# argumentcomputer/lurk-beta

Hardware: NVIDIA H100
Metric: Lurk iterations proved/sec (fib rc=100, Nova IVC) (higher is better)
Workload: dtype u32x8 (254-bit Montgomery integers)

## Files before the change

include/lurk_b200.h:

```cpp
#ifndef LURK_B200_H
#define LURK_B200_H

#include <stddef.h>
#include <stdint.h>

#ifdef __cplusplus
extern "C" {
#endif

#define LURK_FIELD_BN254_FR 0
#define LURK_FIELD_BN254_FQ 1
#define LURK_FIELD_PALLAS_FQ 2
#define LURK_FIELD_PALLAS_FP 3

#define LURK_CURVE_BN254_G1 0
#define LURK_CURVE_GRUMPKIN 1
#define LURK_CURVE_PALLAS 2
#define LURK_CURVE_VESTA 3

#define LURK_FMT_CANONICAL 0
#define LURK_FMT_MONTGOMERY 1

#define LURK_OK 0
#define LURK_ERR_ARG (-1)
// ... 29 lines not shown
int lurk_bitdecomp_witness_batch_dev(int field_id, const void *d_values, size_t n, void *d_blocks, int fmt,
                                     void *stream);

#define LURK_DAG_TUPLE2 2
#define LURK_DAG_TUPLE3 3
#define LURK_DAG_TUPLE4 4
#define LURK_DAG_COMPACT 5
#define LURK_DAG_COMMITMENT 6
typedef struct lurk_dag_node {
    uint8_t kind;
    uint8_t reserved;
    uint16_t tag[4];
    uint32_t child[4];
} lurk_dag_node;
int lurk_dag_hash(int field_id, const lurk_dag_node *nodes, size_t n, const uint8_t *atom_digests,
                  size_t n_atoms, uint8_t *out_digests);
typedef struct lurk_dag_plan {
    uint64_t nodes, levels, max_width;
    uint64_t est_gpu_us;
    uint64_t est_cpu_core_us;
    int use_gpu;
} lurk_dag_plan;
int lurk_dag_hash_plan(const lurk_dag_node *nodes, size_t n, size_t n_atoms, lurk_dag_plan *plan);

typedef struct lurk_msm_ctx lurk_msm_ctx;
int lurk_msm_ctx_create(int curve_id, const uint8_t *bases_affine, size_t n, int fmt, lurk_msm_ctx **out);
int lurk_msm_ctx_create_dev(int curve_id, const void *d_bases_mont, size_t n, lurk_msm_ctx **out);
void lurk_msm_ctx_destroy(lurk_msm_ctx *ctx);
int lurk_msm_ctx_info(lurk_msm_ctx *ctx, int *curve_id, size_t *n);
int lurk_msm_ctx_run(lurk_msm_ctx *ctx, const uint8_t *scalars, size_t n, int fmt, uint8_t out_xyz[96]);
int lurk_msm_ctx_run_dev(lurk_msm_ctx *ctx, const void *d_scalars, size_t n, int fmt, uint8_t out_xyz[96],
                         void *stream);
int lurk_msm_ctx_precompute(lurk_msm_ctx *ctx);
int lurk_msm_ctx_launch_dev(lurk_msm_ctx *ctx, const void *d_scalars, size_t n, int fmt, void *stream);
int lurk_msm_ctx_finish(lurk_msm_ctx *ctx, uint8_t out_xyz[96]);
int lurk_msm_ctx_clone(lurk_msm_ctx *ctx, lurk_msm_ctx **out);
int lurk_msm_ctx_set_profiling(lurk_msm_ctx *ctx, int enable);
int lurk_msm_ctx_last_profile(lurk_msm_ctx *ctx, float *accumulate_ms, unsigned *kernel_launches);
int lurk_msm(int curve_id, const uint8_t *bases_affine, const uint8_t *scalars, size_t n, int fmt,
             uint8_t out_xyz[96]);
int lurk_synthetic_bases(int curve_id, uint64_t start, size_t n, int fmt, uint8_t *bases_out);
int lurk_point_sum(int curve_id, const uint8_t *points_xyz, size_t count, int fmt, uint8_t out_xyz[96]);

size_t lurk_ck_size(size_t num_cons, size_t num_vars, size_t ck_floor);
int lurk_ck_generate(int curve_id, const uint8_t *label, size_t label_len, size_t n, int fmt, uint8_t *bases_out);
int lurk_ck_generate_dev(int curve_id, const uint8_t *label, size_t label_len, size_t n, void *d_bases_mont, void *stream);
int lurk_ck_generate_range_dev(int curve_id, const uint8_t *label, size_t label_len, size_t first, size_t n, void *d_bases_mont,
                               void *stream);
int lurk_hash_to_curve_batch(int curve_id, const char *domain_prefix, const uint8_t *messages, size_t msg_len, size_t n, int fmt,
                             uint8_t *points_out);
int lurk_hash_to_curve_batch_dev(int curve_id, const char *domain_prefix, const void *d_messages, size_t msg_len, size_t n,
                                 void *d_points, int fmt, void *stream);
int lurk_ck_powers_dev(int curve_id, const uint8_t g[64], const uint8_t beta[32], size_t n, void *d_bases_mont, int fmt, void *stream);
int lurk_shake256(const uint8_t *in, size_t in_len, uint8_t *out, size_t out_len);

typedef int (*lurk_challenge_fn)(void *user, int round, const uint8_t *message, size_t message_len, uint8_t challenge_out[32]);
#define LURK_SUMCHECK_QUAD 0
#define LURK_SUMCHECK_CUBIC 1
int lurk_sumcheck_prove_dev(int field_id, int kind, void *const *d_polys, int num_rounds, const uint8_t claim[32],
                            lurk_challenge_fn challenge, void *user, uint8_t *round_evals, uint8_t *challenges, uint8_t *final_evals,
                            int fmt, void *stream);
int lurk_sumcheck_prove_batch_dev(int field_id, int kind, int n_instances, void *const *d_polys, const int *num_rounds,
                                  const uint8_t *claims, const uint8_t *coeffs, lurk_challenge_fn challenge, void *user,
                                  uint8_t *round_evals, uint8_t *challenges, uint8_t *final_evals, int fmt, void *stream);
int lurk_eq_evals_dev(int field_id, const uint8_t *tau, int num_vars, void *d_out, int fmt, void *stream);
int lurk_inner_product_dev(int field_id, const void *d_a, const void *d_b, size_t n, uint8_t out[32], int fmt, void *stream);
int lurk_ipa_fold_scalars_dev(int field_id, void *d_a, size_t n, const uint8_t x[32], const uint8_t y[32], int fmt, void *stream);
int lurk_ipa_fold_bases_dev(int curve_id, void *d_bases_mont, size_t n, const uint8_t x[32], const uint8_t y[32], int fmt, void *stream);
int lurk_ipa_prove_dev(int curve_id, lurk_msm_ctx *ck, const uint8_t ck_c[64], void *d_a, void *d_b, int log_n,
                       lurk_challenge_fn challenge, void *user, uint8_t *L_out, uint8_t *R_out, uint8_t a_final[32], uint8_t b_final[32],
                       int fmt, void *stream);
// ... 199 lines not shown
```

lurk-beta_b200/_capi.py:

```python
import ctypes as C
import os

_HERE = os.path.dirname(os.path.abspath(__file__))
LIB_PATH = os.path.join(_HERE, "liblurk_b200.so")

FIELD_BN254_FR, FIELD_BN254_FQ, FIELD_PALLAS_FQ, FIELD_PALLAS_FP = 0, 1, 2, 3
CURVE_BN254_G1, CURVE_GRUMPKIN, CURVE_PALLAS, CURVE_VESTA = 0, 1, 2, 3
FMT_CANONICAL, FMT_MONTGOMERY = 0, 1
OK, ERR_ARG, ERR_CUDA, ERR_OOM, ERR_RANGE, ERR_NOGPU, ERR_ORDER = 0, -1, -2, -3, -4, -5, -6


class LurkError(RuntimeError):
    def __init__(self, code, msg):
        super().__init__(f"liblurk_b200 error {code}: {msg}")
        self.code = code


class DagNode(C.Structure):
    _fields_ = [("kind", C.c_uint8), ("reserved", C.c_uint8), ("tag", C.c_uint16 * 4), ("child", C.c_uint32 * 4)]


class DagPlan(C.Structure):
    _fields_ = [("nodes", C.c_uint64), ("levels", C.c_uint64), ("max_width", C.c_uint64), ("est_gpu_us", C.c_uint64),
                ("est_cpu_core_us", C.c_uint64), ("use_gpu", C.c_int)]
# ... 67 lines not shown
class RecursiveVerdict(C.Structure):
    _fields_ = [("bad_rows", C.c_uint64), ("first_bad_row", C.c_uint64), ("u_ok", C.c_int), ("comm_W_ok", C.c_int), ("comm_E_ok", C.c_int)]


PROTOTYPES = {
    "lurk_last_error": (C.c_char_p, []),
    "lurk_version": (_i, []),
    "lurk_device_count": (_i, []),
    "lurk_field_modulus": (_i, [_i, _vp]),
    "lurk_poseidon_hash_batch": (_i, [_i, _i, _vp, _sz, _vp]),
    "lurk_poseidon_hash_batch_mont": (_i, [_i, _i, _vp, _sz, _vp]),
    "lurk_poseidon_hash_batch_dev": (_i, [_i, _i, _vp, _sz, _vp, _i, _vp]),
    "lurk_poseidon_constants": (_i, [_i, _i, C.POINTER(_i), C.POINTER(_i), _vp, _vp]),
    "lurk_poseidon_witness_block": (_sz, [_i, _i]),
    "lurk_poseidon_witness_batch": (_i, [_i, _i, _vp, _sz, _vp, _i]),
    "lurk_poseidon_witness_batch_dev": (_i, [_i, _i, _vp, _sz, _vp, _i, _vp]),
    "lurk_poseidon_witness_scatter_dev": (_i, [_i, _i, _vp, _sz, _vp, _vp, _i, _vp]),
    "lurk_bitdecomp_witness_scatter_dev": (_i, [_i, _vp, _sz, _vp, _vp, _i, _vp]),
    "lurk_bitdecomp_witness_block": (_sz, [_i]),
    "lurk_bitdecomp_witness_batch": (_i, [_i, _vp, _sz, _vp, _i]),
    "lurk_bitdecomp_witness_batch_dev": (_i, [_i, _vp, _sz, _vp, _i, _vp]),
    "lurk_dag_hash": (_i, [_i, _vp, _sz, _vp, _sz, _vp]),
    "lurk_dag_hash_plan": (_i, [_vp, _sz, _sz, C.POINTER(DagPlan)]),
    "lurk_msm_ctx_create": (_i, [_i, _vp, _sz, _i, C.POINTER(_vp)]),
    "lurk_msm_ctx_create_dev": (_i, [_i, _vp, _sz, C.POINTER(_vp)]),
    "lurk_msm_ctx_destroy": (None, [_vp]),
    "lurk_msm_ctx_run": (_i, [_vp, _vp, _sz, _i, _vp]),
    "lurk_msm_ctx_run_dev": (_i, [_vp, _vp, _sz, _i, _vp, _vp]),
    "lurk_msm": (_i, [_i, _vp, _vp, _sz, _i, _vp]),
    "lurk_msm_ctx_launch_dev": (_i, [_vp, _vp, _sz, _i, _vp]),
    "lurk_msm_ctx_finish": (_i, [_vp, _vp]),
    "lurk_msm_ctx_clone": (_i, [_vp, C.POINTER(_vp)]),
    "lurk_msm_ctx_precompute": (_i, [_vp]),
    "lurk_msm_ctx_set_profiling": (_i, [_vp, _i]),
    "lurk_msm_ctx_last_profile": (_i, [_vp, C.POINTER(C.c_float), C.POINTER(C.c_uint)]),
    "lurk_point_sum": (_i, [_i, _vp, _sz, _i, _vp]),
    "lurk_synthetic_bases": (_i, [_i, C.c_uint64, _sz, _i, _vp]),
    "lurk_ck_size": (_sz, [_sz, _sz, _sz]),
    "lurk_ck_generate": (_i, [_i, _vp, _sz, _sz, _i, _vp]),
    "lurk_ck_generate_dev": (_i, [_i, _vp, _sz, _sz, _vp, _vp]),
    "lurk_ck_generate_range_dev": (_i, [_i, _vp, _sz, _sz, _sz, _vp, _vp]),
    "lurk_hash_to_curve_batch": (_i, [_i, C.c_char_p, _vp, _sz, _sz, _i, _vp]),
    "lurk_hash_to_curve_batch_dev": (_i, [_i, C.c_char_p, _vp, _sz, _sz, _vp, _i, _vp]),
    "lurk_shake256": (_i, [_vp, _sz, _vp, _sz]),
    "lurk_sumcheck_prove_dev": (_i, [_i, _i, C.POINTER(_vp), _i, _vp, CHALLENGE_FN, _vp, _vp, _vp, _vp, _i, _vp]),
    "lurk_sumcheck_prove_batch_dev": (_i, [_i, _i, _i, C.POINTER(_vp), C.POINTER(_i), _vp, _vp, CHALLENGE_FN, _vp, _vp, _vp, _vp, _i, _vp]),
    "lurk_eq_evals_dev": (_i, [_i, _vp, _i, _vp, _i, _vp]),
    "lurk_inner_product_dev": (_i, [_i, _vp, _vp, _sz, _vp, _i, _vp]),
    "lurk_ipa_fold_scalars_dev": (_i, [_i, _vp, _sz, _vp, _vp, _i, _vp]),
    "lurk_ipa_fold_bases_dev": (_i, [_i, _vp, _sz, _vp, _vp, _i, _vp]),
    "lurk_ipa_prove_dev": (_i, [_i, _vp, _vp, _vp, _vp, _i, CHALLENGE_FN, _vp, _vp, _vp, _vp, _vp, _i, _vp]),
    "lurk_msm_ctx_info": (_i, [_vp, C.POINTER(_i), C.POINTER(_sz)]),
    "lurk_ck_powers_dev": (_i, [_i, _vp, _vp, _sz, _vp, _i, _vp]),
    "lurk_hyperkzg_prove_dev": (_i, [_i, _vp, _vp, _vp, _i, CHALLENGE_FN, _vp, _vp, _vp, _vp, _i, _vp]),
    "lurk_batch_eval_reduce_dev": (_i, [_i, _i, C.POINTER(_vp), C.POINTER(_i), _vp, _vp, CHALLENGE_FN, _vp, _vp, _vp, _vp, _vp, _vp, _vp, _i, _vp]),
    "lurk_spartan_ctx_create": (_i, [_i, C.c_uint64, C.c_uint64, C.c_uint64, C.POINTER(_vp), C.POINTER(_vp), C.POINTER(_vp), _i, C.POINTER(_vp)]),
    "lurk_spartan_ctx_create_verifier": (_i, [_i, C.c_uint64, C.c_uint64, C.c_uint64, C.POINTER(_vp), C.POINTER(_vp), C.POINTER(_vp), _i, C.POINTER(_vp)]),
    "lurk_spartan_ctx_destroy": (None, [_vp]),
    "lurk_spartan_ctx_info": (_i, [_vp, C.POINTER(_i), C.POINTER(_i), C.POINTER(_i), C.POINTER(_sz)]),
    "lurk_spartan_prove_dev": (_i, [_vp, _vp, _vp, SPARTAN_CHALLENGE_FN, _vp, C.POINTER(SpartanProof), _vp, _i, _vp]),
    "lurk_spartan_prove_batch_dev": (_i, [_i, C.POINTER(_vp), C.POINTER(_vp), C.POINTER(_vp), SPARTAN_CHALLENGE_FN, _vp, C.POINTER(SpartanProof), _vp, _i,
                                          _vp]),
    "lurk_spartan_eval_table_dev": (_i, [_vp, _vp, _vp, _vp, _i, _vp]),
    "lurk_spartan_matrix_evals_dev": (_i, [_vp, _vp, _vp, _vp, _i, _vp]),
    "lurk_spartan_verify": (_i, [_vp, _vp, _vp, C.POINTER(SpartanProof), _i, SPARTAN_CHALLENGE_FN, _vp, C.POINTER(_i), _i, _vp]),
    "lurk_spartan_verify_batch": (_i, [_i, C.POINTER(_vp), _vp, C.POINTER(_vp), C.POINTER(SpartanProof), _i, SPARTAN_CHALLENGE_FN, _vp, C.POINTER(_i),
                                       _i, _vp]),
    "lurk_compress_ctx_create": (_i, [_i, C.POINTER(_vp), _vp, C.POINTER(CompressPcs), C.POINTER(CompressPcs), _i, C.POINTER(_vp)]),
# ... 62 lines not shown
```

lurk-beta_b200/commit.py:

```python
import ctypes as C

import numpy as np

from . import _capi


class CommitmentKey:
    def __init__(self, curve_id, bases, fmt=_capi.FMT_CANONICAL):
        self.curve_id = curve_id
        bases = np.ascontiguousarray(bases, dtype=np.uint8).reshape(-1)
        if bases.size % 64:
            raise ValueError("bases buffer is not a whole number of affine points")
        self.n = bases.size // 64
        self._ctx = C.c_void_p()
        _capi.check(_capi.lib().lurk_msm_ctx_create(curve_id, _capi.np_ptr(bases), self.n, fmt, C.byref(self._ctx)))

    @classmethod
    def from_device(cls, curve_id, d_bases_ptr, n):
        self = cls.__new__(cls)
        self.curve_id, self.n = curve_id, n
        self._ctx = C.c_void_p()
        _capi.check(_capi.lib().lurk_msm_ctx_create_dev(curve_id, C.c_void_p(d_bases_ptr), n, C.byref(self._ctx)))
        return self

# ... 7 lines not shown
        self._bases = buf
        return self

    @classmethod
    def powers_of_tau(cls, curve_id, g, beta, n):
        import torch
        buf = torch.empty(max(n, 1) * 64, dtype=torch.uint8, device="cuda")
        gb = np.frombuffer(int(g[0]).to_bytes(32, "little") + int(g[1]).to_bytes(32, "little"), dtype=np.uint8).copy()
        bb = np.frombuffer(int(beta).to_bytes(32, "little"), dtype=np.uint8).copy()
        _capi.check(_capi.lib().lurk_ck_powers_dev(curve_id, _capi.np_ptr(gb), _capi.np_ptr(bb), n, C.c_void_p(buf.data_ptr()), _capi.FMT_CANONICAL, None))
        self = cls.from_device(curve_id, buf.data_ptr(), n)
        self._bases = buf
        return self

    def commit(self, scalars, fmt=_capi.FMT_CANONICAL):
        scalars = np.ascontiguousarray(scalars, dtype=np.uint8).reshape(-1)
        out = np.zeros(96, dtype=np.uint8)
        _capi.check(_capi.lib().lurk_msm_ctx_run(self._ctx, _capi.np_ptr(scalars), scalars.size // 32, fmt, _capi.np_ptr(out)))
        return out

    def commit_device(self, d_scalars_ptr, n, fmt=_capi.FMT_MONTGOMERY, stream=0):
        out = np.zeros(96, dtype=np.uint8)
        _capi.check(_capi.lib().lurk_msm_ctx_run_dev(self._ctx, C.c_void_p(d_scalars_ptr), n, fmt, _capi.np_ptr(out), C.c_void_p(stream)))
        return out

    def launch_device(self, d_scalars_ptr, n, fmt=_capi.FMT_MONTGOMERY, stream=0):
        _capi.check(_capi.lib().lurk_msm_ctx_launch_dev(self._ctx, C.c_void_p(d_scalars_ptr), n, fmt, C.c_void_p(stream)))

    def finish(self):
        out = np.zeros(96, dtype=np.uint8)
        _capi.check(_capi.lib().lurk_msm_ctx_finish(self._ctx, _capi.np_ptr(out)))
        return out

    def precompute(self):
        _capi.check(_capi.lib().lurk_msm_ctx_precompute(self._ctx))
        return self

    def clone(self):
        other = CommitmentKey.__new__(CommitmentKey)
        other.curve_id, other.n, other._parent = self.curve_id, self.n, self
        other._ctx = C.c_void_p()
        _capi.check(_capi.lib().lurk_msm_ctx_clone(self._ctx, C.byref(other._ctx)))
        return other

    def set_profiling(self, enable=True):
        _capi.check(_capi.lib().lurk_msm_ctx_set_profiling(self._ctx, 1 if enable else 0))

    def last_profile(self):
        ms, k = C.c_float(), C.c_uint()
        _capi.check(_capi.lib().lurk_msm_ctx_last_profile(self._ctx, C.byref(ms), C.byref(k)))
        return ms.value, k.value

    def close(self):
        if getattr(self, "_ctx", None) and self._ctx.value:
            _capi.lib().lurk_msm_ctx_destroy(self._ctx)
            self._ctx = C.c_void_p()

    def __del__(self):
        try:
            self.close()
        except Exception:
            pass


def synthetic_bases(curve_id, n, start=0, fmt=_capi.FMT_CANONICAL):
    out = np.zeros(n * 64, dtype=np.uint8)
    _capi.check(_capi.lib().lurk_synthetic_bases(curve_id, start, n, fmt, _capi.np_ptr(out)))
    return out


def ck_size(num_cons, num_vars, ck_floor=0):
    return int(_capi.lib().lurk_ck_size(num_cons, num_vars, ck_floor))


def from_label(curve_id, label, n, fmt=_capi.FMT_CANONICAL):
    out = np.zeros(n * 64, dtype=np.uint8)
    label = bytes(label)
    _capi.check(_capi.lib().lurk_ck_generate(curve_id, label, len(label), n, fmt, _capi.np_ptr(out)))
    return out


def hash_to_curve_batch(curve_id, domain_prefix, messages, msg_len, fmt=_capi.FMT_CANONICAL):
    messages = np.ascontiguousarray(messages, dtype=np.uint8).reshape(-1)
    n = messages.size // msg_len if msg_len else 0
# ... 54 lines not shown
```

lurk-beta_b200/csrc/foldctx_impl.cuh:

```cuda
#pragma once
#include "msm_impl.cuh"
#include "poseidon_api.h"
#include "spmv3.cuh"

#include <memory>
#include <string>

namespace lurk {

static constexpr int FOLD_MAX_WORLD = 16;
static constexpr int FOLD_MAX_DEPTH = 4;
static constexpr int FOLD_MAX_SPANS = 4;
static constexpr int FOLD_RO_RATE = 24;
static constexpr int FOLD_W_WINDOW = 17;
static constexpr int FOLD_T_WINDOW = 16;

template <class F>
__global__ void __launch_bounds__(256) cross_term_dev_kernel(const F *__restrict__ az1, const F *__restrict__ bz1, const F *__restrict__ cz1,
                                                             const F *__restrict__ az2, const F *__restrict__ bz2, const F *__restrict__ cz2,
                                                             const F *__restrict__ u1p, const F *__restrict__ u2p, size_t n, F *__restrict__ t) {
    const F u1 = load_fe<F>(u1p), u2 = load_fe<F>(u2p);
    for (size_t i = (size_t)blockIdx.x * blockDim.x + threadIdx.x; i < n; i += (size_t)gridDim.x * blockDim.x) {
        WideAcc<typename F::Params> acc;
        acc.clear();
        acc.mul_acc(load_fe<F>(az1 + i), load_fe<F>(bz2 + i));
        acc.mul_acc(load_fe<F>(az2 + i), load_fe<F>(bz1 + i));
        F pos = acc.reduce();
        WideAcc<typename F::Params> neg;
        neg.clear();
        neg.mul_acc(u1, load_fe<F>(cz2 + i));
        neg.mul_acc(u2, load_fe<F>(cz1 + i));
        store_fe(t + i, pos - neg.reduce());
    }
}

template <class F>
struct FoldAxpyArgs {
    F *dst[5];
    const F *src[5];
    size_t end[5];
};
template <class F>
__global__ void __launch_bounds__(256) fold_axpy_kernel(FoldAxpyArgs<F> a, const F *__restrict__ rp) {
    const F r = load_fe<F>(rp);
    const size_t total = a.end[4];
    for (size_t i = (size_t)blockIdx.x * blockDim.x + threadIdx.x; i < total; i += (size_t)gridDim.x * blockDim.x) {
        int v = 0;
// ... 365 lines not shown
```

lurk-beta_b200/csrc/msm.cu:

```cuda
#include "msm_impl.cuh"

namespace lurk {
LURK_MSM_EXTERN(CurveBn254G1)
LURK_MSM_EXTERN(CurveGrumpkin)
LURK_MSM_EXTERN(CurvePallas)
LURK_MSM_EXTERN(CurveVesta)
}

using namespace lurk;

extern "C" {

int lurk_msm_ctx_create_dev(int curve_id, const void *d_bases_mont, size_t n, lurk_msm_ctx **out) {
    if (!out) { set_error("null out"); return LURK_ERR_ARG; }
    *out = nullptr;
    if (curve_id < 0 || curve_id > 3) { set_error("unknown curve id %d", curve_id); return LURK_ERR_ARG; }
    if (n >= ((size_t)1 << 31)) { set_error("commitment key too large"); return LURK_ERR_ARG; }
    LURK_TRY(require_gpu());
    lurk_msm_ctx *ctx = new lurk_msm_ctx();
    ctx->curve_id = curve_id;
    ctx->n = n;
    ctx->d_bases = const_cast<void *>(d_bases_mont);
    cudaGetDevice(&ctx->device);
    *out = ctx;
    return LURK_OK;
}

int lurk_msm_ctx_create(int curve_id, const uint8_t *bases_affine, size_t n, int fmt, lurk_msm_ctx **out) {
    if (fmt != LURK_FMT_CANONICAL && fmt != LURK_FMT_MONTGOMERY) { set_error("bad format %d", fmt); return LURK_ERR_ARG; }
    if (n && !bases_affine) { set_error("null bases"); return LURK_ERR_ARG; }
    LURK_TRY(lurk_msm_ctx_create_dev(curve_id, nullptr, n, out));
    if (n == 0) return LURK_OK;
    int rc = dispatch_curve(curve_id, [&](auto c) { return ctx_upload<decltype(c)>(*out, bases_affine, n, fmt); });
    if (rc != LURK_OK) { lurk_msm_ctx_destroy(*out); *out = nullptr; }
    return rc;
}

int lurk_msm_ctx_set_profiling(lurk_msm_ctx *ctx, int enable) {
    if (!ctx) { set_error("null context"); return LURK_ERR_ARG; }
    std::lock_guard<std::mutex> g(ctx->mu);
    if (enable && !ctx->ev0) {
        LURK_CUDA_TRY(cudaEventCreate(&ctx->ev0));
        LURK_CUDA_TRY(cudaEventCreate(&ctx->ev1));
    }
    ctx->profile = enable != 0;
    return LURK_OK;
}
int lurk_msm_ctx_last_profile(lurk_msm_ctx *ctx, float *accumulate_ms, unsigned *kernel_launches) {
    if (!ctx) { set_error("null context"); return LURK_ERR_ARG; }
    if (accumulate_ms) *accumulate_ms = ctx->last_accumulate_ms;
    if (kernel_launches) *kernel_launches = ctx->last_launches;
    return LURK_OK;
}

int lurk_msm_ctx_info(lurk_msm_ctx *ctx, int *curve_id, size_t *n) {
    if (!ctx) { set_error("null context"); return LURK_ERR_ARG; }
    if (curve_id) *curve_id = ctx->curve_id;
    if (n) *n = ctx->n;
    return LURK_OK;
}

void lurk_msm_ctx_destroy(lurk_msm_ctx *ctx) {
    if (!ctx) return;
    if (ctx->ev0) { cudaEventDestroy(ctx->ev0); cudaEventDestroy(ctx->ev1); }
    if (ctx->done) cudaEventDestroy(ctx->done);
    if (ctx->ev_fork) { cudaEventDestroy(ctx->ev_fork); cudaEventDestroy(ctx->ev_join); }
    if (ctx->owns_bases && ctx->d_bases) cudaFree(ctx->d_bases);
    if (ctx->owns_table && ctx->d_table) cudaFree(ctx->d_table);
    delete ctx;
}

int lurk_msm_ctx_run_dev(lurk_msm_ctx *ctx, const void *d_scalars, size_t n, int fmt, uint8_t out_xyz[96], void *stream) {
    if (!ctx || !out_xyz) { set_error("null argument"); return LURK_ERR_ARG; }
    if (fmt != LURK_FMT_CANONICAL && fmt != LURK_FMT_MONTGOMERY) { set_error("bad format %d", fmt); return LURK_ERR_ARG; }
    if (n > ctx->n) { set_error("%zu scalars for a commitment key of %zu bases", n, ctx->n); return LURK_ERR_ARG; }
    std::lock_guard<std::mutex> g(ctx->mu);
    return dispatch_curve(ctx->curve_id, [&](auto c) { return msm_run<decltype(c)>(ctx, d_scalars, n, fmt, out_xyz, (cudaStream_t)stream); });
}

int lurk_msm_ctx_launch_dev(lurk_msm_ctx *ctx, const void *d_scalars, size_t n, int fmt, void *stream) {
    if (!ctx) { set_error("null argument"); return LURK_ERR_ARG; }
    if (fmt != LURK_FMT_CANONICAL && fmt != LURK_FMT_MONTGOMERY) { set_error("bad format %d", fmt); return LURK_ERR_ARG; }
    if (n > ctx->n) { set_error("%zu scalars for a commitment key of %zu bases", n, ctx->n); return LURK_ERR_ARG; }
    std::lock_guard<std::mutex> g(ctx->mu);
    return dispatch_curve(ctx->curve_id, [&](auto c) { return msm_launch<decltype(c)>(ctx, d_scalars, n, fmt, (cudaStream_t)stream, true); });
}
int lurk_msm_ctx_finish(lurk_msm_ctx *ctx, uint8_t out_xyz[96]) {
    if (!ctx || !out_xyz) { set_error("null argument"); return LURK_ERR_ARG; }
    std::lock_guard<std::mutex> g(ctx->mu);
    return dispatch_curve(ctx->curve_id, [&](auto c) { return msm_finish<decltype(c)>(ctx, out_xyz); });
}
int lurk_msm_ctx_precompute(lurk_msm_ctx *ctx) {
    if (!ctx) { set_error("null context"); return LURK_ERR_ARG; }
    std::lock_guard<std::mutex> g(ctx->mu);
    if (ctx->d_table || ctx->n == 0) return LURK_OK;
    if (ctx->pending) { set_error("a launch is pending on this context"); return LURK_ERR_ARG; }
    return dispatch_curve(ctx->curve_id, [&](auto cv) { return msm_precompute<decltype(cv)>(ctx, 0); });
}

int lurk_msm_ctx_clone(lurk_msm_ctx *ctx, lurk_msm_ctx **out) {
    if (!ctx || !out) { set_error("null argument"); return LURK_ERR_ARG; }
    std::lock_guard<std::mutex> g(ctx->mu);
    lurk_msm_ctx *c = new lurk_msm_ctx();
    c->curve_id = ctx->curve_id;
    c->device = ctx->device;
    c->n = ctx->n;
    c->d_bases = ctx->d_bases;
    c->owns_bases = false;
    c->d_table = ctx->d_table;
    c->owns_table = false;
    c->fixed_c = ctx->fixed_c;
    *out = c;
    return LURK_OK;
}

int lurk_msm_ctx_run(lurk_msm_ctx *ctx, const uint8_t *scalars, size_t n, int fmt, uint8_t out_xyz[96]) {
    if (!ctx || !out_xyz || (n && !scalars)) { set_error("null argument"); return LURK_ERR_ARG; }
    if (n > ctx->n) { set_error("%zu scalars for a commitment key of %zu bases", n, ctx->n); return LURK_ERR_ARG; }
    if (n == 0) { memset(out_xyz, 0, 96); return LURK_OK; }
    if (fmt != LURK_FMT_CANONICAL && fmt != LURK_FMT_MONTGOMERY) { set_error("bad format %d", fmt); return LURK_ERR_ARG; }
    std::lock_guard<std::mutex> g(ctx->mu);
    if (ctx->pending) { set_error("a launch is already pending on this context (call lurk_msm_ctx_finish)"); return LURK_ERR_ARG; }
    LURK_TRY(ctx_check_device(ctx));
    if (ctx->scratch.scalars.bytes < n * 32) LURK_TRY(ctx->scratch.scalars.alloc(n * 32));
    MsmScratch &S = ctx->scratch;
    const size_t STAGE = (size_t)8 << 20;
    if (!S.stage_stream) LURK_CUDA_TRY(cudaStreamCreateWithFlags(&S.stage_stream, cudaStreamNonBlocking));
    cudaStream_t hs = S.stage_stream;
    if (!S.h_stage[0]) {
        for (int k = 0; k < 2; k++) {
// ... 98 lines not shown
```

lurk-beta_b200/csrc/msm_impl.cuh:

```cuda
#pragma once
#include "common.cuh"

#include <algorithm>
#include <atomic>
#include <mutex>
#include <thread>

namespace lurk {

static constexpr uint32_t KEY_NONE = 0xffffffffu;

struct MsmPlan {
    int c = 0;
    int nwin = 0;
    uint32_t nb = 0;
    uint32_t total_buckets = 0;
    uint32_t seg = 0;
    uint32_t t1 = 0;
    bool fixed = false;
    uint32_t rwin = 0, K = 0, G = 0, nq = 0, SL = 0, slice = 0;
};
static constexpr uint32_t MSM_MAX_RESULT_POINTS = 512;

inline int fixed_base_window(size_t key_n) {
// ... 135 lines not shown
template <class Fs>
__global__ void __launch_bounds__(256) msm_scatter_kernel(const Fs *__restrict__ scalars, const Fs *__restrict__ sub, size_t n, int fmt, int c, int nwin,
                                                          uint32_t key_stride, uint32_t base_stride, const uint32_t *__restrict__ offsets,
                                                          uint32_t *__restrict__ cursor, uint32_t *__restrict__ sorted) {
    size_t i = (size_t)blockIdx.x * blockDim.x + threadIdx.x;
    const bool live = i < n;
    Fs k = Fs::zero();
    if (live) {
        k = load_fe<Fs>(scalars + i);
        if (sub) k = k - load_fe<Fs>(sub + i);
        if (fmt == LURK_FMT_MONTGOMERY) k = k.to_canonical();
    }
    uint32_t carry = 0;
    const uint32_t half = 1u << (c - 1);
    const uint32_t lane = threadIdx.x & 31;
    for (int w = 0; w < nwin; w++) {
        uint32_t raw = window_bits(k.v, w * c, c) + carry;
        uint32_t neg = raw > half;
        uint32_t mag = neg ? (1u << c) - raw : raw;
        carry = neg;
        uint32_t key = (live && mag) ? (uint32_t)w * key_stride + (mag - 1) : KEY_NONE;
        uint32_t peers = __match_any_sync(0xffffffffu, key);
        uint32_t leader = (uint32_t)(__ffs(peers) - 1);
        uint32_t base = 0;
        if (key != KEY_NONE && lane == leader) base = atomicAdd(cursor + key, (uint32_t)__popc(peers));
        base = __shfl_sync(0xffffffffu, base, leader);
        if (key != KEY_NONE) {
            uint32_t rank = __popc(peers & ((1u << lane) - 1));
            sorted[offsets[key] + base + rank] = ((uint32_t)i + (uint32_t)w * base_stride) | (neg << 31);
        }
    }
}

template <class Fb>
__device__ __forceinline__ Affine<Fb> load_affine(const Affine<Fb> *p) {
    Affine<Fb> a;
    a.x = load_fe<Fb>(&p->x);
    a.y = load_fe<Fb>(&p->y);
    return a;
}
template <class Fb>
__device__ __forceinline__ XYZZ<Fb> load_xyzz(const XYZZ<Fb> *p) {
    XYZZ<Fb> a;
    a.x = load_fe<Fb>(&p->x); a.y = load_fe<Fb>(&p->y); a.zz = load_fe<Fb>(&p->zz); a.zzz = load_fe<Fb>(&p->zzz);
    return a;
}
template <class Fb>
__device__ __forceinline__ void store_xyzz(XYZZ<Fb> *p, const XYZZ<Fb> &a) {
    store_fe(&p->x, a.x); store_fe(&p->y, a.y); store_fe(&p->zz, a.zz); store_fe(&p->zzz, a.zzz);
}

template <class Fb, int MINB, bool DIRECT = false>
__global__ void __launch_bounds__(128, MINB) msm_accumulate_kernel(const uint32_t *__restrict__ offsets, uint32_t nbuckets,
                                                             const uint32_t *__restrict__ sorted, const Affine<Fb> *__restrict__ bases,
                                                             XYZZ<Fb> *__restrict__ bucket_acc, XYZZ<Fb> *__restrict__ ppt, uint32_t seg,
                                                             uint32_t nthreads) {
    const uint32_t t = blockIdx.x * blockDim.x + threadIdx.x;
    if (t >= nthreads) return;
    const uint32_t total = offsets[nbuckets];
    const uint64_t start64 = (uint64_t)t * seg;
    if (start64 >= total) return;
    const uint32_t start = (uint32_t)start64;
    const uint32_t end = (uint32_t)min((uint64_t)total, start64 + seg);
    uint32_t lo = 0, hi = nbuckets;
    while (hi - lo > 1) {
        uint32_t mid = (lo + hi) >> 1;
// ... 307 lines not shown
        a.y = Fb::zero();
        if (!pts[w].is_identity()) {
            const Fb zi = inv * pref[w];
            inv = inv * pts[w].zzz;
            const Fb zz_inv = (zi * pts[w].zz).sqr();
            a.x = pts[w].x * zz_inv;
            a.y = pts[w].y * zi;
        }
        store_fe(&table[(size_t)w * n + i].x, a.x);
        store_fe(&table[(size_t)w * n + i].y, a.y);
    }
}

template <class Fb>
__global__ void __launch_bounds__(256) msm_on_curve_kernel(const Affine<Fb> *__restrict__ bases, size_t n, Fb b, int *bad) {
    int local = 0;
    for (size_t i = (size_t)blockIdx.x * blockDim.x + threadIdx.x; i < n; i += (size_t)gridDim.x * blockDim.x) {
        const Affine<Fb> p = load_affine(bases + i);
        if (p.is_identity()) continue;
        const Fb lhs = p.y.sqr(), rhs = p.x.sqr() * p.x + b;
        local += lhs == rhs ? 0 : 1;
    }
    local = __reduce_add_sync(0xffffffffu, local);
    if ((threadIdx.x & 31) == 0 && local) atomicAdd(bad, local);
}

template <class Fb>
__global__ void __launch_bounds__(256) msm_bases_to_mont_kernel(Fb *coords, size_t count) {
    for (size_t i = (size_t)blockIdx.x * blockDim.x + threadIdx.x; i < count; i += (size_t)gridDim.x * blockDim.x)
        store_fe(coords + i, Fb::from_canonical(load_fe<Fb>(coords + i)));
}

struct MsmScratch {
    DevBuf counts, offsets, tiles, sorted, buckets, ppt, chunks, chunk_sums, slices, wins, result, scalars, pair_offs[2], pair_pts[2];
    void *h_wins = nullptr;
    void *h_stage[2] = {nullptr, nullptr};
    cudaEvent_t stage_done[2] = {nullptr, nullptr};
    cudaStream_t stage_stream = nullptr;
    ~MsmScratch() {
        if (h_wins) cudaFreeHost(h_wins);
        if (stage_stream) cudaStreamDestroy(stage_stream);
        for (int k = 0; k < 2; k++) { if (h_stage[k]) cudaFreeHost(h_stage[k]); if (stage_done[k]) cudaEventDestroy(stage_done[k]); }
    }
};

}

using namespace lurk;

struct lurk_msm_ctx {
    int curve_id = 0;
    int device = 0;
    size_t n = 0;
    void *d_bases = nullptr;
    bool owns_bases = false;
    void *d_table = nullptr;
    bool owns_table = false;
    int fixed_c = 0;
    std::mutex mu;
    MsmScratch scratch;
    bool profile = false;
    cudaEvent_t ev0 = nullptr, ev1 = nullptr;
    float last_accumulate_ms = 0.f;
    unsigned last_launches = 0;
    bool pending = false;
    int pending_fmt = 0, pending_c = 0, pending_nwin = 0;
    bool pending_fixed = false;
    uint32_t pending_nq = 0, pending_K = 0;
    cudaEvent_t done = nullptr;
    cudaStream_t tiny_stream = nullptr;
    const void *d_sub = nullptr;
    const void *d_offset = nullptr;
    cudaEvent_t ev_fork = nullptr, ev_join = nullptr;
};

namespace lurk {

template <class Fb>
void point_to_bytes(const XYZZ<Fb> &p, int fmt, uint8_t out[96]) {
    memset(out, 0, 96);
    if (p.is_identity()) return;
    Affine<Fb> a = p.to_affine();
    Fb one = Fb::one();
    if (fmt == LURK_FMT_CANONICAL) { a.x = a.x.to_canonical(); a.y = a.y.to_canonical(); one = one.to_canonical(); }
    memcpy(out, a.x.v, 32); memcpy(out + 32, a.y.v, 32); memcpy(out + 64, one.v, 32);
}

inline int ctx_check_device(const lurk_msm_ctx *ctx) {
    int dev = -1;
    LURK_CUDA_TRY(cudaGetDevice(&dev));
    if (dev != ctx->device) { set_error("context belongs to device %d but device %d is current", ctx->device, dev); return LURK_ERR_ARG; }
    return LURK_OK;
}

template <class C>
// ... 4 lines not shown
    if (ctx->pending) { set_error("a launch is already pending on this context (call lurk_msm_ctx_finish)"); return LURK_ERR_ARG; }
    LURK_TRY(ctx_check_device(ctx));
    if (!ctx->done) LURK_CUDA_TRY(cudaEventCreateWithFlags(&ctx->done, cudaEventDisableTiming));
    ctx->pending_fmt = fmt;
    ctx->pending_nwin = 0;
    MsmScratch &S = ctx->scratch;
    if (S.result.bytes < sizeof(Pt)) LURK_TRY(S.result.alloc(sizeof(Pt)));
    if (n == 0) {
        if (readback) ctx->pending = true;
        else LURK_CUDA_TRY(cudaMemsetAsync(S.result.p, 0, sizeof(Pt), s));
        return LURK_OK;
    }
    const bool table_pays = !readback || n * (size_t)(Fs::Params::NBITS / std::max(ctx->fixed_c, 1) + 1) >= ((size_t)8 << (std::max(ctx->fixed_c, 1) - 1));
    const bool fixed = ctx->d_table != nullptr && table_pays;
    if (!readback && !fixed) { set_error("device-resident results need the fixed-base table (lurk_msm_ctx_precompute)"); return LURK_ERR_ARG; }
    MsmPlan P = make_plan(n, Fs::Params::NBITS, fixed ? ctx->fixed_c : 0);
    if ((uint64_t)n * (uint64_t)P.nwin >= (1ull << 32)) { set_error("%zu scalars exceed one launch (shard the commitment key)", n); return LURK_ERR_ARG; }
    const uint32_t TB = P.total_buckets;
    const uint32_t ntiles = (TB + SCAN_TILE - 1) / SCAN_TILE;
    const size_t cap = n * (size_t)P.nwin;
    int rounds = 0;
    {
        static const int forced = [] { const char *e = getenv("LURK_MSM_PAIR_ROUNDS"); return e ? atoi(e) : -1; }();
        const size_t avg = cap / TB;
        if (forced >= 0) rounds = forced;
        else if (n >= 8192) rounds = avg >= 12 ? MSM_PAIR_ROUNDS_LONG : (avg >= 5 ? MSM_PAIR_ROUNDS_SHORT : 0);
        if (rounds > 4) rounds = 4;
    }
    size_t cap_final = cap;
    for (int r = 0; r < rounds; r++) cap_final = cap_final / 2 + TB + 1;
    const uint32_t t1 = rounds ? (uint32_t)((cap_final + P.seg - 1) / P.seg) : P.t1;
    const uint32_t t1_alloc = std::max(t1, P.t1);
    const uint32_t max_long = t1 / (MSM_LONG_PARTIALS + 1) + 1;
    {
        auto ensure = [](DevBuf &b, size_t bytes) { return b.bytes >= bytes ? LURK_OK : b.alloc(bytes); };
        LURK_TRY(ensure(S.counts, (((size_t)TB + 1) * 2 + 1 + max_long) * sizeof(uint32_t)));
        LURK_TRY(ensure(S.offsets, ((size_t)TB + 1) * sizeof(uint32_t)));
        LURK_TRY(ensure(S.tiles, ((size_t)ntiles + 1) * 2 * sizeof(uint32_t)));
        LURK_TRY(ensure(S.sorted, n * (size_t)P.nwin * sizeof(uint32_t)));
        LURK_TRY(ensure(S.buckets, (size_t)TB * sizeof(Pt)));
        LURK_TRY(ensure(S.ppt, (size_t)t1_alloc * sizeof(Pt)));
        const size_t nchunks_all = (size_t)P.rwin * P.G;
        LURK_TRY(ensure(S.chunks, nchunks_all * sizeof(Pt)));
        LURK_TRY(ensure(S.chunk_sums, nchunks_all * sizeof(Pt)));
        LURK_TRY(ensure(S.slices, (size_t)P.rwin * P.nq * P.SL * sizeof(Pt)));
        LURK_TRY(ensure(S.wins, MSM_MAX_RESULT_POINTS * sizeof(Pt)));
        if (!S.h_wins) LURK_CUDA_TRY(cudaMallocHost(&S.h_wins, MSM_MAX_RESULT_POINTS * sizeof(Pt)));
    }
    if (ntiles > 4096) { set_error("bucket table too large for the scan"); return LURK_ERR_ARG; }
    uint32_t *counts = S.counts.as<uint32_t>();
    uint32_t *cursor = counts + (TB + 1);
    uint32_t *offsets = S.offsets.as<uint32_t>();
    uint32_t *tile_sums = S.tiles.as<uint32_t>(), *tile_offsets = tile_sums + (ntiles + 1);
    uint32_t *sorted = S.sorted.as<uint32_t>();
    uint32_t *long_list = cursor + (TB + 1) + 1;
    Pt *buckets = S.buckets.as<Pt>();

    LURK_CUDA_TRY(cudaMemsetAsync(counts, 0, (((size_t)TB + 1) * 2 + 1) * sizeof(uint32_t), s));
    const unsigned gs = (unsigned)((n + 255) / 256);
    unsigned launches = 0;
    const uint32_t key_stride = fixed ? 0u : P.nb;
    const uint32_t base_stride = fixed ? (uint32_t)ctx->n : 0u;
    const Affine<Fb> *bases = (const Affine<Fb> *)(fixed ? ctx->d_table : ctx->d_bases);
    const Fs *sub = (!readback && fmt == LURK_FMT_MONTGOMERY) ? (const Fs *)ctx->d_sub : nullptr;
    msm_count_kernel<Fs><<<gs, 256, 0, s>>>((const Fs *)d_scalars, sub, n, fmt, P.c, P.nwin, key_stride, counts);
    msm_scan_tile_sums_kernel<<<ntiles, 1024, 0, s>>>(counts, TB, tile_sums);
    msm_scan_tiles_kernel<<<1, 1024, 0, s>>>(tile_sums, ntiles, tile_offsets);
    msm_scan_apply_kernel<<<ntiles, 1024, 0, s>>>(counts, TB, tile_offsets, ntiles, offsets, P.seg, rounds ? nullptr : long_list);
    msm_scatter_kernel<Fs><<<gs, 256, 0, s>>>((const Fs *)d_scalars, sub, n, fmt, P.c, P.nwin, key_stride, base_stride, offsets, cursor, sorted);
    if (ctx->profile) LURK_CUDA_TRY(cudaEventRecord(ctx->ev0, s));
    const uint32_t *acc_offs = offsets;
    const Affine<Fb> *acc_pts = bases;
    size_t cap_r = cap;
    for (int r = 0; r < rounds; r++) {
        cap_r = cap_r / 2 + TB + 1;
        DevBuf &ob = S.pair_offs[r & 1], &pb = S.pair_pts[r & 1];
        if (ob.bytes < ((size_t)TB + 1) * sizeof(uint32_t)) LURK_TRY(ob.alloc(((size_t)TB + 1) * sizeof(uint32_t)));
        if (pb.bytes < cap_r * sizeof(Affine<Fb>)) LURK_TRY(pb.alloc(cap_r * sizeof(Affine<Fb>)));
        uint32_t *o2 = ob.as<uint32_t>();
        msm_halve_kernel<<<(TB + 256) / 256, 256, 0, s>>>(acc_offs, TB, counts);
        msm_scan_tile_sums_kernel<<<ntiles, 1024, 0, s>>>(counts, TB, tile_sums);
        msm_scan_tiles_kernel<<<1, 1024, 0, s>>>(tile_sums, ntiles, tile_offsets);
        msm_scan_apply_kernel<<<ntiles, 1024, 0, s>>>(counts, TB, tile_offsets, ntiles, o2, P.seg, r == rounds - 1 ? long_list : nullptr);
        const size_t pthreads = (cap_r + PAIR_B - 1) / PAIR_B;
        const unsigned pgrid = (unsigned)((pthreads + 127) / 128);
        if (r == 0) msm_pair_kernel<Fb, true><<<pgrid, 128, 0, s>>>(acc_offs, o2, TB, sorted, acc_pts, pb.as<Affine<Fb>>());
        else msm_pair_kernel<Fb, false><<<pgrid, 128, 0, s>>>(acc_offs, o2, TB, sorted, acc_pts, pb.as<Affine<Fb>>());
        launches += 5;
        acc_offs = o2;
        acc_pts = pb.as<Affine<Fb>>();
    }
    if (rounds)
        msm_accumulate_kernel<Fb, 5, true><<<(t1 + 127) / 128, 128, 0, s>>>(acc_offs, TB, sorted, acc_pts, buckets, S.ppt.as<Pt>(), P.seg, t1);
    else if (fixed)
        msm_accumulate_kernel<Fb, 5><<<(P.t1 + 127) / 128, 128, 0, s>>>(offsets, TB, sorted, bases, buckets, S.ppt.as<Pt>(), P.seg, P.t1);
    else
        msm_accumulate_kernel<Fb, 4><<<(P.t1 + 127) / 128, 128, 0, s>>>(offsets, TB, sorted, bases, buckets, S.ppt.as<Pt>(), P.seg, P.t1);
    if (ctx->profile) LURK_CUDA_TRY(cudaEventRecord(ctx->ev1, s));
    launches += 6;
    msm_merge_long_kernel<Fb><<<std::min<uint32_t>(max_long, 2 * sm_count()), MSM_MERGE_LONG_THREADS, 0, s>>>(acc_offs, P.seg, S.ppt.as<Pt>(),
                                                                                                             long_list, buckets);
    msm_merge_kernel<Fb><<<(TB + MSM_MERGE_THREADS - 1) / MSM_MERGE_THREADS, MSM_MERGE_THREADS, 0, s>>>(acc_offs, TB, P.seg, S.ppt.as<Pt>(), buckets);
// ... 138 lines not shown
```

Baseline: 23510.

## Use shared-memory per-CTA histogram bucket sort for fixed-base MSM

For fixed-base MSM contexts, the global-atomic count and scatter kernels are replaced with per-CTA shared-memory histograms. A column-wise prefix kernel combines them, and the scatter uses shared-memory cursors, so global atomic contention on bucket counters goes away. The fold witness window shrinks from 17 to 16 bits, which halves the bucket table and lets it fit in shared memory. The change also adds a precompute-with-window API and sort-time profiling, and the new path adds an extra per-CTA histogram buffer and a kernel launch.

```diff
diff --git a/include/lurk_b200.h b/include/lurk_b200.h
--- a/include/lurk_b200.h
+++ b/include/lurk_b200.h
@@ -85,11 +85,13 @@
 int lurk_msm_ctx_run_dev(lurk_msm_ctx *ctx, const void *d_scalars, size_t n, int fmt, uint8_t out_xyz[96],
                          void *stream);
 int lurk_msm_ctx_precompute(lurk_msm_ctx *ctx);
+int lurk_msm_ctx_precompute_window(lurk_msm_ctx *ctx, int c);
 int lurk_msm_ctx_launch_dev(lurk_msm_ctx *ctx, const void *d_scalars, size_t n, int fmt, void *stream);
 int lurk_msm_ctx_finish(lurk_msm_ctx *ctx, uint8_t out_xyz[96]);
 int lurk_msm_ctx_clone(lurk_msm_ctx *ctx, lurk_msm_ctx **out);
 int lurk_msm_ctx_set_profiling(lurk_msm_ctx *ctx, int enable);
 int lurk_msm_ctx_last_profile(lurk_msm_ctx *ctx, float *accumulate_ms, unsigned *kernel_launches);
+int lurk_msm_ctx_last_sort_ms(lurk_msm_ctx *ctx, float *sort_ms);
 int lurk_msm(int curve_id, const uint8_t *bases_affine, const uint8_t *scalars, size_t n, int fmt,
              uint8_t out_xyz[96]);
 int lurk_synthetic_bases(int curve_id, uint64_t start, size_t n, int fmt, uint8_t *bases_out);
diff --git a/lurk-beta_b200/_capi.py b/lurk-beta_b200/_capi.py
--- a/lurk-beta_b200/_capi.py
+++ b/lurk-beta_b200/_capi.py
@@ -123,8 +123,10 @@
     "lurk_msm_ctx_finish": (_i, [_vp, _vp]),
     "lurk_msm_ctx_clone": (_i, [_vp, C.POINTER(_vp)]),
     "lurk_msm_ctx_precompute": (_i, [_vp]),
+    "lurk_msm_ctx_precompute_window": (_i, [_vp, _i]),
     "lurk_msm_ctx_set_profiling": (_i, [_vp, _i]),
     "lurk_msm_ctx_last_profile": (_i, [_vp, C.POINTER(C.c_float), C.POINTER(C.c_uint)]),
+    "lurk_msm_ctx_last_sort_ms": (_i, [_vp, C.POINTER(C.c_float)]),
     "lurk_point_sum": (_i, [_i, _vp, _sz, _i, _vp]),
     "lurk_synthetic_bases": (_i, [_i, C.c_uint64, _sz, _i, _vp]),
     "lurk_ck_size": (_sz, [_sz, _sz, _sz]),
diff --git a/lurk-beta_b200/commit.py b/lurk-beta_b200/commit.py
--- a/lurk-beta_b200/commit.py
+++ b/lurk-beta_b200/commit.py
@@ -63,8 +63,11 @@
         _capi.check(_capi.lib().lurk_msm_ctx_finish(self._ctx, _capi.np_ptr(out)))
         return out
 
-    def precompute(self):
-        _capi.check(_capi.lib().lurk_msm_ctx_precompute(self._ctx))
+    def precompute(self, window=0):
+        if window:
+            _capi.check(_capi.lib().lurk_msm_ctx_precompute_window(self._ctx, window))
+        else:
+            _capi.check(_capi.lib().lurk_msm_ctx_precompute(self._ctx))
         return self
 
     def clone(self):
@@ -81,6 +84,11 @@
         ms, k = C.c_float(), C.c_uint()
         _capi.check(_capi.lib().lurk_msm_ctx_last_profile(self._ctx, C.byref(ms), C.byref(k)))
         return ms.value, k.value
+
+    def last_sort_ms(self):
+        ms = C.c_float()
+        _capi.check(_capi.lib().lurk_msm_ctx_last_sort_ms(self._ctx, C.byref(ms)))
+        return ms.value
 
     def close(self):
         if getattr(self, "_ctx", None) and self._ctx.value:
diff --git a/lurk-beta_b200/csrc/foldctx_impl.cuh b/lurk-beta_b200/csrc/foldctx_impl.cuh
--- a/lurk-beta_b200/csrc/foldctx_impl.cuh
+++ b/lurk-beta_b200/csrc/foldctx_impl.cuh
@@ -12,7 +12,7 @@
 static constexpr int FOLD_MAX_DEPTH = 4;
 static constexpr int FOLD_MAX_SPANS = 4;
 static constexpr int FOLD_RO_RATE = 24;
-static constexpr int FOLD_W_WINDOW = 17;
+static constexpr int FOLD_W_WINDOW = 16;
 static constexpr int FOLD_T_WINDOW = 16;
 
 template <class F>
diff --git a/lurk-beta_b200/csrc/msm.cu b/lurk-beta_b200/csrc/msm.cu
--- a/lurk-beta_b200/csrc/msm.cu
+++ b/lurk-beta_b200/csrc/msm.cu
@@ -42,6 +42,7 @@
     if (enable && !ctx->ev0) {
         LURK_CUDA_TRY(cudaEventCreate(&ctx->ev0));
         LURK_CUDA_TRY(cudaEventCreate(&ctx->ev1));
+        LURK_CUDA_TRY(cudaEventCreate(&ctx->ev_sort));
     }
     ctx->profile = enable != 0;
     return LURK_OK;
@@ -50,6 +51,15 @@
     if (!ctx) { set_error("null context"); return LURK_ERR_ARG; }
     if (accumulate_ms) *accumulate_ms = ctx->last_accumulate_ms;
     if (kernel_launches) *kernel_launches = ctx->last_launches;
+    return LURK_OK;
+}
+
+int lurk_msm_ctx_last_sort_ms(lurk_msm_ctx *ctx, float *sort_ms) {
+    if (!ctx || !sort_ms) { set_error("null argument"); return LURK_ERR_ARG; }
+    std::lock_guard<std::mutex> g(ctx->mu);
+    *sort_ms = 0.f;
+    if (ctx->pending) { set_error("a launch is pending on this context"); return LURK_ERR_ARG; }
+    if (ctx->ev_sort) LURK_CUDA_TRY(cudaEventElapsedTime(sort_ms, ctx->ev_sort, ctx->ev0));
     return LURK_OK;
 }
 
@@ -63,6 +73,7 @@
 void lurk_msm_ctx_destroy(lurk_msm_ctx *ctx) {
     if (!ctx) return;
     if (ctx->ev0) { cudaEventDestroy(ctx->ev0); cudaEventDestroy(ctx->ev1); }
+    if (ctx->ev_sort) cudaEventDestroy(ctx->ev_sort);
     if (ctx->done) cudaEventDestroy(ctx->done);
     if (ctx->ev_fork) { cudaEventDestroy(ctx->ev_fork); cudaEventDestroy(ctx->ev_join); }
     if (ctx->owns_bases && ctx->d_bases) cudaFree(ctx->d_bases);
@@ -96,6 +107,16 @@
     if (ctx->d_table || ctx->n == 0) return LURK_OK;
     if (ctx->pending) { set_error("a launch is pending on this context"); return LURK_ERR_ARG; }
     return dispatch_curve(ctx->curve_id, [&](auto cv) { return msm_precompute<decltype(cv)>(ctx, 0); });
+}
+
+int lurk_msm_ctx_precompute_window(lurk_msm_ctx *ctx, int c) {
+    if (!ctx) { set_error("null context"); return LURK_ERR_ARG; }
+    std::lock_guard<std::mutex> g(ctx->mu);
+    if (ctx->d_table) { set_error("the context already has a fixed-base table"); return LURK_ERR_ARG; }
+    if (ctx->n == 0) return LURK_OK;
+    if (ctx->pending) { set_error("a launch is pending on this context"); return LURK_ERR_ARG; }
+    if (c <= 0) { set_error("window width %d out of range", c); return LURK_ERR_ARG; }
+    return dispatch_curve(ctx->curve_id, [&](auto cv) { return msm_precompute<decltype(cv)>(ctx, c); });
 }
 
 int lurk_msm_ctx_clone(lurk_msm_ctx *ctx, lurk_msm_ctx **out) {
diff --git a/lurk-beta_b200/csrc/msm_impl.cuh b/lurk-beta_b200/csrc/msm_impl.cuh
--- a/lurk-beta_b200/csrc/msm_impl.cuh
+++ b/lurk-beta_b200/csrc/msm_impl.cuh
@@ -191,6 +191,82 @@
     }
 }
 
+static constexpr uint32_t MSM_SORT_THREADS = 1024;
+static constexpr size_t MSM_SORT_SMEM_MAX = (size_t)128 << 10;
+
+template <class Fs>
+__device__ __forceinline__ bool sort_scalar(const Fs *__restrict__ scalars, const Fs *__restrict__ sub, size_t i, int fmt, Fs &k) {
+    k = load_fe<Fs>(scalars + i);
+    if (sub) k = k - load_fe<Fs>(sub + i);
+    if (k.is_zero()) return false;
+    if (fmt == LURK_FMT_MONTGOMERY) k = k.to_canonical();
+    return true;
+}
+
+template <class Fs>
+__global__ void __launch_bounds__(MSM_SORT_THREADS) msm_hist_smem_kernel(const Fs *__restrict__ scalars, const Fs *__restrict__ sub, size_t n, int fmt, int c,
+                                                                         int nwin, uint32_t nb, uint32_t *__restrict__ cnt) {
+    extern __shared__ uint32_t sort_smem[];
+    for (uint32_t b = threadIdx.x; b < nb; b += MSM_SORT_THREADS) sort_smem[b] = 0;
+    __syncthreads();
+    const size_t lo = (size_t)blockIdx.x * n / gridDim.x, hi = (size_t)(blockIdx.x + 1) * n / gridDim.x;
+    const uint32_t half = 1u << (c - 1);
+    for (size_t i = lo + threadIdx.x; i < hi; i += MSM_SORT_THREADS) {
+        Fs k;
+        if (!sort_scalar(scalars, sub, i, fmt, k)) continue;
+        uint32_t carry = 0;
+        for (int w = 0; w < nwin; w++) {
+            const uint32_t raw = window_bits(k.v, w * c, c) + carry;
+            carry = raw > half;
+            const uint32_t mag = carry ? (1u << c) - raw : raw;
+            if (mag) atomicAdd(sort_smem + (mag - 1), 1u);
+        }
+    }
+    __syncthreads();
+    uint32_t *row = cnt + (size_t)blockIdx.x * nb;
+    for (uint32_t b = threadIdx.x; b < nb; b += MSM_SORT_THREADS) row[b] = sort_smem[b];
+}
+
+static __global__ void __launch_bounds__(256) msm_hist_columns_kernel(uint32_t *__restrict__ cnt, uint32_t G, uint32_t nb, uint32_t *__restrict__ counts) {
+    const uint32_t b = blockIdx.x * blockDim.x + threadIdx.x;
+    if (b >= nb) return;
+    uint32_t run = 0;
+    for (uint32_t g0 = 0; g0 < G; g0 += 8) {
+        uint32_t v[8];
+#pragma unroll
+        for (uint32_t j = 0; j < 8; j++) v[j] = g0 + j < G ? cnt[(size_t)(g0 + j) * nb + b] : 0u;
+#pragma unroll
+        for (uint32_t j = 0; j < 8; j++) {
+            if (g0 + j < G) cnt[(size_t)(g0 + j) * nb + b] = run;
+            run += v[j];
+        }
+    }
+    counts[b] = run;
+}
+
+template <class Fs>
+__global__ void __launch_bounds__(MSM_SORT_THREADS) msm_scatter_smem_kernel(const Fs *__restrict__ scalars, const Fs *__restrict__ sub, size_t n, int fmt, int c,
+                                                                            int nwin, uint32_t nb, uint32_t base_stride, const uint32_t *__restrict__ offsets,
+                                                                            const uint32_t *__restrict__ cnt, uint32_t *__restrict__ sorted) {
+    extern __shared__ uint32_t sort_smem[];
+    const uint32_t *row = cnt + (size_t)blockIdx.x * nb;
+    for (uint32_t b = threadIdx.x; b < nb; b += MSM_SORT_THREADS) sort_smem[b] = offsets[b] + row[b];
+    __syncthreads();
+    const size_t lo = (size_t)blockIdx.x * n / gridDim.x, hi = (size_t)(blockIdx.x + 1) * n / gridDim.x;
+    const uint32_t half = 1u << (c - 1);
+    for (size_t i = lo + threadIdx.x; i < hi; i += MSM_SORT_THREADS) {
+        Fs k;
+        if (!sort_scalar(scalars, sub, i, fmt, k)) continue;
+        uint32_t carry = 0;
+        for (int w = 0; w < nwin; w++) {
+            const uint32_t raw = window_bits(k.v, w * c, c) + carry;
+            carry = raw > half;
+            const uint32_t mag = carry ? (1u << c) - raw : raw;
+            if (mag) sorted[atomicAdd(sort_smem + (mag - 1), 1u)] = ((uint32_t)i + (uint32_t)w * base_stride) | (carry << 31);
+        }
+    }
+}
+
 template <class Fb>
 __device__ __forceinline__ Affine<Fb> load_affine(const Affine<Fb> *p) {
     Affine<Fb> a;
@@ -564,7 +640,7 @@
 }
 
 struct MsmScratch {
-    DevBuf counts, offsets, tiles, sorted, buckets, ppt, chunks, chunk_sums, slices, wins, result, scalars, pair_offs[2], pair_pts[2];
+    DevBuf counts, hist, offsets, tiles, sorted, buckets, ppt, chunks, chunk_sums, slices, wins, result, scalars, pair_offs[2], pair_pts[2];
     void *h_wins = nullptr;
     void *h_stage[2] = {nullptr, nullptr};
     cudaEvent_t stage_done[2] = {nullptr, nullptr};
@@ -592,7 +668,7 @@
     std::mutex mu;
     MsmScratch scratch;
     bool profile = false;
-    cudaEvent_t ev0 = nullptr, ev1 = nullptr;
+    cudaEvent_t ev0 = nullptr, ev1 = nullptr, ev_sort = nullptr;
     float last_accumulate_ms = 0.f;
     unsigned last_launches = 0;
     bool pending = false;
@@ -663,9 +739,13 @@
     const uint32_t t1 = rounds ? (uint32_t)((cap_final + P.seg - 1) / P.seg) : P.t1;
     const uint32_t t1_alloc = std::max(t1, P.t1);
     const uint32_t max_long = t1 / (MSM_LONG_PARTIALS + 1) + 1;
+    const char *sort_env = getenv("LURK_MSM_SORT");
+    const bool smem_sort = fixed && (size_t)P.nb * sizeof(uint32_t) <= MSM_SORT_SMEM_MAX && !(sort_env && !strcmp(sort_env, "legacy"));
+    const uint32_t sort_ctas = (uint32_t)std::min<size_t>((size_t)sm_count(), (n + MSM_SORT_THREADS - 1) / MSM_SORT_THREADS);
     {
         auto ensure = [](DevBuf &b, size_t bytes) { return b.bytes >= bytes ? LURK_OK : b.alloc(bytes); };
         LURK_TRY(ensure(S.counts, (((size_t)TB + 1) * 2 + 1 + max_long) * sizeof(uint32_t)));
+        if (smem_sort) LURK_TRY(ensure(S.hist, (size_t)sort_ctas * P.nb * sizeof(uint32_t)));
         LURK_TRY(ensure(S.offsets, ((size_t)TB + 1) * sizeof(uint32_t)));
         LURK_TRY(ensure(S.tiles, ((size_t)ntiles + 1) * 2 * sizeof(uint32_t)));
         LURK_TRY(ensure(S.sorted, n * (size_t)P.nwin * sizeof(uint32_t)));
@@ -687,18 +767,35 @@
     uint32_t *long_list = cursor + (TB + 1) + 1;
     Pt *buckets = S.buckets.as<Pt>();
 
-    LURK_CUDA_TRY(cudaMemsetAsync(counts, 0, (((size_t)TB + 1) * 2 + 1) * sizeof(uint32_t), s));
-    const unsigned gs = (unsigned)((n + 255) / 256);
+    if (ctx->profile) LURK_CUDA_TRY(cudaEventRecord(ctx->ev_sort, s));
     unsigned launches = 0;
     const uint32_t key_stride = fixed ? 0u : P.nb;
     const uint32_t base_stride = fixed ? (uint32_t)ctx->n : 0u;
     const Affine<Fb> *bases = (const Affine<Fb> *)(fixed ? ctx->d_table : ctx->d_bases);
     const Fs *sub = (!readback && fmt == LURK_FMT_MONTGOMERY) ? (const Fs *)ctx->d_sub : nullptr;
-    msm_count_kernel<Fs><<<gs, 256, 0, s>>>((const Fs *)d_scalars, sub, n, fmt, P.c, P.nwin, key_stride, counts);
+    if (smem_sort) {
+        const size_t smem = (size_t)P.nb * sizeof(uint32_t);
+        uint32_t *cnt = S.hist.as<uint32_t>();
+        if (smem > ((size_t)48 << 10)) {
+            LURK_CUDA_TRY(cudaFuncSetAttribute(msm_hist_smem_kernel<Fs>, cudaFuncAttributeMaxDynamicSharedMemorySize, (int)smem));
+            LURK_CUDA_TRY(cudaFuncSetAttribute(msm_scatter_smem_kernel<Fs>, cudaFuncAttributeMaxDynamicSharedMemorySize, (int)smem));
+        }
+        LURK_CUDA_TRY(cudaMemsetAsync(long_list - 1, 0, sizeof(uint32_t), s));
+        msm_hist_smem_kernel<Fs><<<sort_ctas, MSM_SORT_THREADS, smem, s>>>((const Fs *)d_scalars, sub, n, fmt, P.c, P.nwin, P.nb, cnt);
+        msm_hist_columns_kernel<<<(P.nb + 255) / 256, 256, 0, s>>>(cnt, sort_ctas, P.nb, counts);
+        launches++;
+    } else {
+        LURK_CUDA_TRY(cudaMemsetAsync(counts, 0, (((size_t)TB + 1) * 2 + 1) * sizeof(uint32_t), s));
+        msm_count_kernel<Fs><<<(unsigned)((n + 255) / 256), 256, 0, s>>>((const Fs *)d_scalars, sub, n, fmt, P.c, P.nwin, key_stride, counts);
+    }
     msm_scan_tile_sums_kernel<<<ntiles, 1024, 0, s>>>(counts, TB, tile_sums);
     msm_scan_tiles_kernel<<<1, 1024, 0, s>>>(tile_sums, ntiles, tile_offsets);
     msm_scan_apply_kernel<<<ntiles, 1024, 0, s>>>(counts, TB, tile_offsets, ntiles, offsets, P.seg, rounds ? nullptr : long_list);
-    msm_scatter_kernel<Fs><<<gs, 256, 0, s>>>((const Fs *)d_scalars, sub, n, fmt, P.c, P.nwin, key_stride, base_stride, offsets, cursor, sorted);
+    if (smem_sort)
+        msm_scatter_smem_kernel<Fs><<<sort_ctas, MSM_SORT_THREADS, (size_t)P.nb * sizeof(uint32_t), s>>>((const Fs *)d_scalars, sub, n, fmt, P.c, P.nwin, P.nb, base_stride,
+                                                                                                       offsets, S.hist.as<uint32_t>(), sorted);
+    else
+        msm_scatter_kernel<Fs><<<(unsigned)((n + 255) / 256), 256, 0, s>>>((const Fs *)d_scalars, sub, n, fmt, P.c, P.nwin, key_stride, base_stride, offsets, cursor, sorted);
     if (ctx->profile) LURK_CUDA_TRY(cudaEventRecord(ctx->ev0, s));
     const uint32_t *acc_offs = offsets;
     const Affine<Fb> *acc_pts = bases;
```

Measured after the change: 24490 (median of 6 runs). 1.04x the previous value.
